# jimouris/draft-mouris-cfrg-mastic

Measured on AMD Instinct MI355X. Metric: VIDPF report x prefix evals/sec at 1/2/4/8 GPUs; % of int-VALU peak, higher is better.
Workload: dtype u32

## Files before the change

draft-mouris-cfrg-mastic_amd/csrc/kernels.hpp:

```cpp
#pragma once
#include "aes.hpp"
#include "flp.hpp"
#include "keccak.hpp"

enum PfxId {
    PFX_EXT = 0,
    PFX_CONV,
    PFX_NODE,
    PFX_ONEHOT,
    PFX_PAYLOAD,
    PFX_EVAL,
    PFX_QUERY,
    PFX_PROOF_SHARE,
    PFX_JR_PART,
    PFX_JR_SEED,
    PFX_JR,
    PFX_PROVE_RAND,
    PFX_TREE,
    PFX_COUNT
};

struct PrefixState {
    KState st;
    int f;
// ... 461 lines not shown
    uint32_t* cache_out;
    int cache_stride;
    uint32_t* wp_buf;
    int recompute_wp;
    int in_stride;
    int fuse_proofs;
    int cur_path_bytes;
    const uint32_t* cur_child_path;
    uint32_t* cur_onehot;
    int pv_level;
    int pv_nodes;
    int pv_npw;
    int pv_path_bytes;
    const uint32_t* pv_child_path;
    uint32_t* pv_onehot;
    int oh_gstride;
    int bin_rstride;
    int pay_gstride;
    const PrefixState* np;
    int np_f;
    int aes_waves;
    int par_waves;
    int proof_prio;
    int aes_prio;
    int dbg_skip;
};

template <class F>
MH_D void parent_payload(const AesPerm& TL, const RkLds& rkc, const uint32_t cv[4], uint32_t t, const uint32_t* cw,
                         int S, int r, int e_lo, int e_hi, uint32_t* out, int row0, int force_slow_blk,
// ... 143 lines not shown
        if (a.proof_prio == 1) __builtin_amdgcn_s_setprio(1);
        if (a.proof_prio == 2) __builtin_amdgcn_s_setprio(2);
        const int nbeg = (blockIdx.y * (EVAL_WAVES - aes_waves) + (wave - aes_waves)) * a.pv_npw;
        const int nend = min(nbeg + a.pv_npw, a.pv_nodes);
        const int pl_ = a.pv_level;
        uint32_t* ohg = a.pv_onehot + (size_t)blockIdx.x * a.oh_gstride;
        const uint32_t lt = (uint32_t)lane * 4u;
        uint32_t pcw[8];
        if constexpr (!WIDE) {
#pragma unroll
            for (int j = 0; j < 8; j++) pcw[j] = pld(pl.cw_proof + ((size_t)pl_ * 8 + j) * S, lb);
        }
        for (int node = nbeg; node < nend; node++) {
            uint32_t sd[4];
#pragma unroll
            for (int i = 0; i < 4; i++) sd[i] = pld(a.cs_in + ((size_t)node * 5 + i) * S_in, lb);
            if constexpr (WIDE) {
                uint32_t w8[8];
                node_proof_one<true>(a.np, a.np_f, p.bits, pl_, a.pv_path_bytes, sd, a.pv_child_path + node * 8, 0u, pcw,
                                     [&](int j, uint32_t w) { w8[j] = w; });
                const uint32_t t = pld(a.cs_in + ((size_t)node * 5 + 4) * S_in, lb);
#pragma unroll
                for (int j = 0; j < 8; j++) pcw[j] = pld(pl.cw_proof + ((size_t)pl_ * 8 + j) * S, lb);
#pragma unroll
                for (int j = 0; j < 8; j++)
                    pst(ohg + ((size_t)node * 8 + j) * a.bin_rstride, lt, w8[j] ^ (t ? pcw[j] : 0u));
            } else {
                const uint32_t t = pld(a.cs_in + ((size_t)node * 5 + 4) * S_in, lb);
                node_proof_one<FC>(a.np, a.np_f, p.bits, pl_, a.pv_path_bytes, sd, a.pv_child_path + node * 8, t, pcw,
                                   [&](int j, uint32_t w) { pst(ohg + ((size_t)node * 8 + j) * a.bin_rstride, lt, w); });
            }
        }
        if (a.proof_prio) __builtin_amdgcn_s_setprio(0);
    }
    const int wp0 = blockIdx.y * a.par_waves * a.ppw;
    const int wp1 = min(wp0 + a.par_waves * a.ppw, SPLIT ? a.n_parents * a.split : a.n_parents);
    const int pn_beg = 2 * wp0, pn_end = 2 * wp1;
    const bool fuse_ovl = FC && a.fuse_proofs == 1;
    auto parent_marked = [&](int q) -> bool {
        const uint32_t w = __hip_atomic_load(parent_done + (q >> 5), __ATOMIC_ACQUIRE, __HIP_MEMORY_SCOPE_WORKGROUP);
        return (__builtin_amdgcn_readfirstlane(w) >> (q & 31)) & 1u;
    };
    auto claim_node = [&]() -> int {
// ... 828 lines not shown
```

draft-mouris-cfrg-mastic_amd/csrc/mastic_hip.hip:

```cpp
#include "mastic_hip.h"

#include <dlfcn.h>
#include <rccl/rccl.h>

#include <algorithm>
#include <atomic>
#include <chrono>
#include <condition_variable>
#include <cstdarg>
#include <cstdio>
#include <cstring>
#include <map>
#include <memory>
#include <mutex>
#include <string>
#include <system_error>
#include <thread>
#include <type_traits>
#include <vector>

#include "comm_agree.hpp"
#include "host_tree.hpp"
#include "kernels.hpp"
#include "shard.hpp"
// ... 158 lines not shown
    int aes_prio = 0;
    int dbg_skip = 0;
    int stride_pad = 64;
    size_t work_arena = (size_t)48 << 30;
    size_t work_arena_fc = (size_t)128 << 30;
    bool binder_tiled = true;
    int absorb_threads = 256;
    int absorb_prio = 3;
    int absorb_dbg = 0;
    int force_slow_blk = -1;
    int fail_allocs = 0;
    int sponge_delay_us = 0;
    int wall_khz = 100000;
    bool timing_nowait = false;
    bool serial_sponges = false;
    bool inject_alloc_failure() {
        if (fail_allocs <= 0) return false;
        fail_allocs--;
        return true;
    }
    bool idle() {
        return hipStreamSynchronize(stream) == hipSuccess && hipStreamSynchronize(stream2) == hipSuccess &&
               hipStreamSynchronize(stream3) == hipSuccess && hipStreamSynchronize(stream4) == hipSuccess;
    }
    int split_sponges = -1;
    bool fuse_last_miss = false;
    bool fuse_last_miss_fc = true;
    bool hit_absorb_main = true;
    bool fc_all = false;
    bool small_split = true;
// ... 430 lines not shown
    const int epb = p.field == 64 ? 2 : 1;
    const int nblk = (p.value_len + epb - 1) / epb;
    const double proofs = 2.0 + (has_prev ? 2.0 * np_prev / std::max(1, np_last) : 0.0);
    const double K = 1585.0 * proofs, A = (4.0 + 2.0 * nblk) * 532.0;
    return std::max(1, std::min(12, (int)std::lround(EVAL_WAVES * K / (K + A))));
}

static int hit_proof_waves(const McParams& p, const mastic_ctx* c) {
    if (c->hit_proof_waves > 0) return c->hit_proof_waves;
    const int epb = p.field == 64 ? 2 : 1;
    const int nblk = (p.value_len + epb - 1) / epb;
    const double K = 3170.0, A = (4.0 + 3.0 * nblk) * 532.0;
    return std::max(1, std::min(12, (int)std::lround(EVAL_WAVES * K / (K + A))));
}

template <class F>
static int run_chunk(mastic_ctx* c, mastic_reports* rep, const Tree* t, const WorkLayout& wl, int agg_id,
                     size_t base, int n, int stride, size_t& evi, LevelCache* lc, bool hit, const uint32_t* cin,
                     uint32_t* cout, uint32_t* W, hipStream_t ss, hipStream_t tail, size_t sev0) {
    const McParams& p = c->p;
    Planes pl = make_planes(W, wl, n, stride);
    Result& R = c->res[agg_id];
    const bool direct = lc && base == 0 && (size_t)n == rep->n && lc->S == (size_t)stride;
    if (direct) {
        pl.sp_onehot = lc->sp.as<uint32_t>();
        pl.sp_payload = lc->sp.as<uint32_t>() + (size_t)50 * lc->S;
        pl.rootsum = lc->rootsum.as<uint32_t>();
    }
    if (hit)
        HIPCHK(c, hipMemsetAsync(pl.status, 0, (size_t)stride * 4, c->stream));
// ... 55 lines not shown
    HIPCHK(c, hipGetLastError());

    const int groups = (n + 63) / 64;
    const int wlw = p.value_len * p.w32;
    int f_oh = c->pfx_f[PFX_ONEHOT], f_pl = c->pfx_f[PFX_PAYLOAD];
    auto plane = [&](size_t off) { return W + off * (size_t)stride; };
    size_t sev = sev0;
    std::vector<hipEvent_t> abs_done(t->L + 1);
    const int oh_gstride = c->binder_tiled ? t->max_level_nodes * 8 * 64 : 64;
    const int pay_gstride = c->binder_tiled ? t->max_parents * wlw * 64 : 64;
    const int bin_rstride = c->binder_tiled ? 64 : stride;
    auto oh_buf = [&](int lv) -> uint32_t* { return plane(wl.onehot[lv % NSLOT]); };
    auto pay_buf = [&](int lv) -> uint32_t* { return plane(wl.payload[lv % NSLOT]); };
    auto oh_gs = [&](int) -> int { return oh_gstride; };
    auto pay_gs = [&](int) -> int { return pay_gstride; };
    const bool pair = c->absorb_mode == 2 || (c->absorb_mode == 0 && (size_t)n < c->absorb_single_min);
    const bool wide = pair && c->eval_wide;
    auto launch_sponges = [&](int lv, int which0, int nwh, hipEvent_t ready, hipEvent_t e4, hipEvent_t e5,
                              hipStream_t as, hipEvent_t* done) -> int {
        AbsorbArgs ab;
        ab.which0 = which0;
        ab.seg[0] = oh_buf(lv);
        ab.gstride[0] = oh_gs(lv);
        ab.nbytes[0] = 2 * t->n_parents[lv] * 32;
        ab.f[0] = f_oh;
        ab.seg[1] = pay_buf(lv);
        ab.gstride[1] = pay_gs(lv);
        ab.rstride = bin_rstride;
        ab.nbytes[1] = lv > 0 ? t->n_parents[lv] * wlw * 4 : 0;
        ab.f[1] = f_pl;
        ab.prio = c->absorb_prio;
        ab.dbg = c->absorb_dbg;
        if (as != c->stream) HIPCHK(c, hipStreamWaitEvent(as, ready, 0));
        if (e4) HIPCHK(c, hipEventRecord(e4, as));
        if (c->dbg_skip & 4) {
        } else if (pair)
            hipLaunchKernelGGL(k_absorb_pair,
                               dim3((groups * 64 * 2 + c->absorb_threads - 1) / c->absorb_threads, (unsigned)nwh),
                               dim3(c->absorb_threads), c->absorb_lds, as, pl, ab);
        else
            hipLaunchKernelGGL(k_absorb, dim3((groups * 64 + 255) / 256, (unsigned)nwh), dim3(256), c->absorb_lds, as,
                               pl, ab);
        if (e5) HIPCHK(c, hipEventRecord(e5, as));
        HIPCHK(c, hipGetLastError());
// ... 23 lines not shown
    if (hit && !direct) {
        if (from_cache(pl.sp_onehot, lc->sp.as<uint32_t>(), 50)) return -1;
        if (from_cache(pl.sp_payload, lc->sp.as<uint32_t>() + (size_t)50 * lc->S, 50)) return -1;
        if (from_cache(pl.rootsum, lc->rootsum.as<uint32_t>(), (size_t)wlw)) return -1;
    }
    if (hit) {
        for (int lv = 0; lv < t->L; lv++) {
            f_oh = (f_oh + 2 * t->n_parents[lv] * 32) % KECCAK_RATE;
            f_pl = (f_pl + (lv > 0 ? t->n_parents[lv] * wlw * 4 : 0)) % KECCAK_RATE;
        }
    }
    const bool fuse_last = hit ? c->fuse_proofs >= 1
                               : ((lc && (c->fuse_proofs == 2 || (c->fuse_proofs >= 1 && c->fuse_last_miss_fc))) ||
                                  (c->fuse_last_miss && c->fuse_proofs >= 1));
    const hipStream_t last_as = (hit && tail == c->stream && c->hit_absorb_main) ? c->stream : ss;
    for (int l = hit ? t->L : 0; l <= t->L; l++) {
        const int np_ = t->n_parents[l];
        if (!hit && l >= NSLOT) {
            HIPCHK(c, hipStreamWaitEvent(c->stream, abs_done[l - NSLOT], 0));
            if (split && pl_done[l - NSLOT]) HIPCHK(c, hipStreamWaitEvent(c->stream, pl_done[l - NSLOT], 0));
        }
        AesArgs a;
        a.level = l;
        a.agg_id = agg_id;
        a.n_parents = np_;
        const int par_waves = c->par_waves > 0 ? c->par_waves : EVAL_WAVES - c->proof_waves;
        a.split = 1;
        a.split_blocks = 0;
        {
            const int epb = p.field == 64 ? 2 : 1;
// ... 31 lines not shown
        if (fuse && a.fuse_proofs == 1)
            a.aes_waves = EVAL_WAVES - (hit ? hit_proof_waves(p, c) : miss_proof_waves(p, c, t->n_parents[l - 1 < 0 ? 0 : l - 1],
                                                                                      np_, l > 0));
        a.par_waves = par_waves;
        a.proof_prio = c->proof_prio;
        a.aes_prio = c->aes_prio;
        a.dbg_skip = c->dbg_skip;
        const int gy = (n_items + a.par_waves * a.ppw - 1) / (a.par_waves * a.ppw);
        a.pv_level = l - 1;
        a.pv_nodes = (l > 0 && !hit) ? 2 * t->n_parents[l - 1] : 0;
        const int pw = EVAL_WAVES - a.aes_waves;
        a.pv_npw = (a.pv_nodes + gy * pw - 1) / (gy * pw);
        a.pv_path_bytes = (l + 7) / 8;
        a.pv_child_path = l > 0 ? t->d_path + t->off[l - 1] * 8 : nullptr;
        a.pv_onehot = l > 0 ? oh_buf(l - 1) : nullptr;
        a.oh_gstride = l > 0 ? oh_gs(l - 1) : oh_gstride;
        a.pay_gstride = pay_gs(l);
        a.bin_rstride = bin_rstride;
        a.np = (const PrefixState*)c->pfx.p + PFX_NODE;
        a.np_f = c->pfx_f[PFX_NODE];
        dim3 grid(groups, gy);
        hipEvent_t e0 = get_event(c, evi++), e1 = get_event(c, evi++);
        hipEvent_t e2 = get_event(c, evi++), e3 = get_event(c, evi++);
        hipEvent_t e4 = get_event(c, evi++), e5 = get_event(c, evi++);
        HIPCHK(c, hipEventRecord(e0, c->stream));
        if ((lc && (hit || l == t->L || c->fc_all)) || fuse)
            hipLaunchKernelGGL((k_eval_aes<F, true, true>), grid, dim3(64 * EVAL_WAVES), EVAL_LDS_BYTES, c->stream,
                               p, pl, a);
        else if (wide && a.split > 1 && l == 0)
            hipLaunchKernelGGL((k_eval_aes_wide<F, true, true>), grid, dim3(64 * EVAL_WAVES), EVAL_LDS_BYTES,
                               c->stream, p, pl, a);
        else if (wide && a.split > 1)
            hipLaunchKernelGGL((k_eval_aes_wide<F, false, true>), grid, dim3(64 * EVAL_WAVES), EVAL_LDS_BYTES,
                               c->stream, p, pl, a);
        else if (wide && (l == 0 || l == t->L))
            hipLaunchKernelGGL((k_eval_aes_wide<F, true>), grid, dim3(64 * EVAL_WAVES), EVAL_LDS_BYTES, c->stream,
                               p, pl, a);
        else if (wide)
            hipLaunchKernelGGL((k_eval_aes_wide<F, false>), grid, dim3(64 * EVAL_WAVES), EVAL_LDS_BYTES, c->stream,
                               p, pl, a);
        else if (a.split > 1 && l == 0)
            hipLaunchKernelGGL((k_eval_aes<F, true, false, true>), grid, dim3(64 * EVAL_WAVES), EVAL_LDS_BYTES,
                               c->stream, p, pl, a);
        else if (a.split > 1)
            hipLaunchKernelGGL((k_eval_aes<F, false, false, true>), grid, dim3(64 * EVAL_WAVES), EVAL_LDS_BYTES,
                               c->stream, p, pl, a);
        else if (l == 0 || l == t->L)
            hipLaunchKernelGGL((k_eval_aes<F, true, false>), grid, dim3(64 * EVAL_WAVES), EVAL_LDS_BYTES, c->stream,
                               p, pl, a);
        else
            hipLaunchKernelGGL((k_eval_aes<F, false, false>), grid, dim3(64 * EVAL_WAVES), EVAL_LDS_BYTES, c->stream,
                               p, pl, a);
        HIPCHK(c, hipEventRecord(e1, c->stream));
        HIPCHK(c, hipGetLastError());
        HIPCHK(c, hipEventRecord(e2, c->stream));
        HIPCHK(c, hipEventRecord(e3, c->stream));
        hipEvent_t aes_done = get_sync_event(c, sev++);
        HIPCHK(c, hipEventRecord(aes_done, c->stream));
        if (split && l > 0) {
            if (launch_sponges(l, 1, 1, aes_done, e4, e5, c->stream3, &pl_done[l])) return -1;
            if (launch_sponges(l - 1, 0, 1, aes_done, nullptr, nullptr, ss, &abs_done[l - 1])) return -1;
        } else if (l > 0 && !hit) {
            if (launch_absorb(l - 1, aes_done, e4, e5, ss)) return -1;
        } else {
            if (c->sponge_delay_us > 0) {
                const unsigned long long ticks =
                    (unsigned long long)c->sponge_delay_us * (unsigned long long)c->wall_khz / 1000;
                c->sponge_delay_us = 0;
                hipLaunchKernelGGL(k_spin, dim3(1), dim3(64), 0, ss, ticks);
                HIPCHK(c, hipGetLastError());
            }
            HIPCHK(c, hipEventRecord(e4, ss));
            HIPCHK(c, hipEventRecord(e5, ss));
        }
    }
    if (fuse_last) {
        const int l = t->L;
        hipEvent_t e0 = get_event(c, evi++), e1 = get_event(c, evi++);
        hipEvent_t e2 = get_event(c, evi++), e3 = get_event(c, evi++);
        hipEvent_t e4 = get_event(c, evi++), e5 = get_event(c, evi++);
        HIPCHK(c, hipEventRecord(e0, c->stream));
        HIPCHK(c, hipEventRecord(e1, c->stream));
        HIPCHK(c, hipEventRecord(e2, c->stream));
        HIPCHK(c, hipEventRecord(e3, c->stream));
        hipEvent_t np_done = get_sync_event(c, sev++);
        HIPCHK(c, hipEventRecord(np_done, c->stream));
        if (split ? launch_sponges(l, 0, 1, np_done, e4, e5, last_as, &abs_done[l])
                  : launch_absorb(l, np_done, e4, e5, last_as))
            return -1;
    } else {
        const int l = t->L;
        const int nn = 2 * t->n_parents[l];
        ProofArgs pa;
        pa.level = l;
        pa.n_nodes = nn;
        pa.npw = choose_ppw(nn, groups);
        pa.path_bytes = (l + 1 + 7) / 8;
        pa.child_path = t->d_path + t->off[l] * 8;
        pa.cs = plane(wl.cs[l & 1]);
        pa.onehot = oh_buf(l);
        pa.oh_gstride = oh_gs(l);
        pa.bin_rstride = bin_rstride;
        pa.np = (const PrefixState*)c->pfx.p + PFX_NODE;
        pa.f = c->pfx_f[PFX_NODE];
        hipEvent_t e0 = get_event(c, evi++), e1 = get_event(c, evi++);
        hipEvent_t e2 = get_event(c, evi++), e3 = get_event(c, evi++);
        hipEvent_t e4 = get_event(c, evi++), e5 = get_event(c, evi++);
        HIPCHK(c, hipEventRecord(e0, c->stream));
        HIPCHK(c, hipEventRecord(e1, c->stream));
        HIPCHK(c, hipEventRecord(e2, c->stream));
        hipLaunchKernelGGL(k_node_proof, dim3(groups, (nn + 4 * pa.npw - 1) / (4 * pa.npw)), dim3(256), 0,
                           c->stream, p, pl, pa);
        HIPCHK(c, hipEventRecord(e3, c->stream));
        HIPCHK(c, hipGetLastError());
        hipEvent_t np_done = get_sync_event(c, sev++);
        HIPCHK(c, hipEventRecord(np_done, c->stream));
        if (split ? launch_sponges(l, 0, 1, np_done, e4, e5, last_as, &abs_done[l])
                  : launch_absorb(l, np_done, e4, e5, last_as))
            return -1;
    }
    hipEvent_t flp_done = nullptr;
    if (t->weight_check) {
        hipEvent_t lv_done = get_sync_event(c, sev++);
        HIPCHK(c, hipEventRecord(lv_done, c->stream));
        HIPCHK(c, hipStreamWaitEvent(c->stream4, lv_done, 0));
        FlpArgs fl{agg_id, t->L};
        hipLaunchKernelGGL(k_flp_rand<F>, dim3((stride + 255) / 256), dim3(256), 0, c->stream4, p, pl, fl, pfx);
        hipLaunchKernelGGL(k_flp_query<F>, dim3((stride + 255) / 256), dim3(256), 0, c->stream4, p, pl,
                           flp_consts<F>(p));
        HIPCHK(c, hipGetLastError());
        flp_done = get_sync_event(c, sev++);
        HIPCHK(c, hipEventRecord(flp_done, c->stream4));
    }
    if (tail != last_as) HIPCHK(c, hipStreamWaitEvent(tail, abs_done[t->L], 0));
    if (split && pl_done[t->L]) HIPCHK(c, hipStreamWaitEvent(tail, pl_done[t->L], 0));
    FinalArgs fa{agg_id, f_oh, f_pl};
    hipLaunchKernelGGL(k_finalize<F>, dim3((stride + 255) / 256), dim3(256), 0, tail, p, pl, fa, pfx);
    HIPCHK(c, hipGetLastError());
    if (flp_done) HIPCHK(c, hipStreamWaitEvent(tail, flp_done, 0));
    if (lc && !direct) {
        if (!hit && to_cache(lc->rootsum.as<uint32_t>(), pl.rootsum, (size_t)wlw)) return -1;
        if (to_cache(lc->sp.as<uint32_t>(), pl.sp_onehot, 50)) return -1;
        if (to_cache(lc->sp.as<uint32_t>() + (size_t)50 * lc->S, pl.sp_payload, 50)) return -1;
    }
    int rc = 0;
    rc |= copy_planes(c, R.eval_proof, R.stride, base, pl.eval_proof, stride, n, 8, tail);
    rc |= copy_planes(c, R.status, R.stride, base, (const uint32_t*)pl.status, stride, n, 1, tail);
    if (t->weight_check) {
        rc |= copy_planes(c, R.verifier, R.stride, base, pl.verifier, stride, n, (size_t)p.verifier_len * p.w32,
                          tail);
// ... 153 lines not shown
            if (c->graveyard.empty() || !c->idle())
                return fail(c, MASTIC_ENOMEM, "out of device memory (work %zu bytes)", want);
            c->bury();
            if (!c->work.ensure(arena) && !c->work.ensure(want))
                return fail(c, MASTIC_ENOMEM, "out of device memory (work %zu bytes)", want);
        }
        chunk = std::min<size_t>(round_up(n, 64), (c->work.bytes / per_report - pad) / 64 * 64);
    }
    if (c->budget) chunk = std::min(chunk, std::max<size_t>(by_budget, 64));
    const bool capped = c->chunk_max > 0 && round_up(c->chunk_max, 64) < chunk;
    if (capped) chunk = round_up(c->chunk_max, 64);
    const size_t half_cap = c->work.bytes / 2 / per_report;
    const bool pipe = c->chunk_pipeline && n > chunk && chunk >= 128 && half_cap >= pad + 64;
    if (pipe) chunk = std::min(capped ? chunk : chunk / 2, half_cap - pad) / 64 * 64;
    const size_t half = c->work.bytes / 2 / 4 / 64 * 64;
    const size_t nsev = 3 * (size_t)t->L + 12;
    size_t evi = 0;
    hipEvent_t t0 = get_event(c, evi++), t1 = get_event(c, evi++);
    HIPCHK(c, hipEventRecord(t0, c->stream));
    hipEvent_t half_free[2] = {get_sync_event(c, 2 * nsev), get_sync_event(c, 2 * nsev + 1)};
    size_t k = 0;
    for (size_t b = 0; b < n; b += chunk, k++) {
        const int nn = (int)std::min(chunk, n - b);
        const int stride = (int)(round_up(nn, 64) + pad);
        const int h = pipe ? (int)(k & 1) : 0;
        if (pipe && k >= 2) HIPCHK(c, hipStreamWaitEvent(c->stream, half_free[h], 0));
        uint32_t* W = c->work.as<uint32_t>() + h * half;
        hipStream_t ss = (pipe && h) ? c->stream3 : c->stream2;
        hipStream_t tail = pipe ? ss : c->stream;
        rc = p.field == 64
                 ? run_chunk<F64>(c, rep, t, wl, agg_id, b, nn, stride, evi, lc, hit, cin, cout, W, ss, tail,
// ... 1079 lines not shown
        if (spl) c->split_sponges = spl[0] == '1' ? 1 : 0;
        const char* flm = getenv("MASTIC_FUSE_LAST_MISS");
        if (flm) c->fuse_last_miss = flm[0] == '1';
        const char* flf = getenv("MASTIC_FUSE_LAST_MISS_FC");
        if (flf) c->fuse_last_miss_fc = flf[0] != '0';
        const char* ham = getenv("MASTIC_HIT_ABSORB_MAIN");
        if (ham) c->hit_absorb_main = ham[0] != '0';
        const char* ssp = getenv("MASTIC_SMALL_SPLIT");
        if (ssp) c->small_split = ssp[0] != '0';
        const char* evw = getenv("MASTIC_EVAL_WIDE");
        if (evw) c->eval_wide = evw[0] != '0';
        const char* tnw = getenv("MASTIC_DBG_TIMING_NOWAIT");
        if (tnw) c->timing_nowait = tnw[0] == '1';
        const char* ssr = getenv("MASTIC_SERIAL_SPONGES");
        if (ssr) c->serial_sponges = ssr[0] == '1';
    }
#endif
    if (hipFuncSetAttribute((const void*)k_eval_aes<F64, false, false>, hipFuncAttributeMaxDynamicSharedMemorySize,
                            EVAL_LDS_BYTES) != hipSuccess ||
        hipFuncSetAttribute((const void*)k_eval_aes<F128, false, false>, hipFuncAttributeMaxDynamicSharedMemorySize,
                            EVAL_LDS_BYTES) != hipSuccess ||
        hipFuncSetAttribute((const void*)k_eval_aes<F64, true, false>, hipFuncAttributeMaxDynamicSharedMemorySize,
                            EVAL_LDS_BYTES) != hipSuccess ||
        hipFuncSetAttribute((const void*)k_eval_aes<F128, true, false>, hipFuncAttributeMaxDynamicSharedMemorySize,
                            EVAL_LDS_BYTES) != hipSuccess ||
        hipFuncSetAttribute((const void*)k_eval_aes<F64, true, true>, hipFuncAttributeMaxDynamicSharedMemorySize,
                            EVAL_LDS_BYTES) != hipSuccess ||
        hipFuncSetAttribute((const void*)k_eval_aes<F128, true, true>, hipFuncAttributeMaxDynamicSharedMemorySize,
                            EVAL_LDS_BYTES) != hipSuccess ||
        hipFuncSetAttribute((const void*)k_eval_aes<F64, true, false, true>,
// ... 80 lines not shown
extern "C" int mastic_set_test_hooks(mastic_ctx* c, int force_slow_blk, int fail_allocs) {
    if (!c) return MASTIC_EINVAL;
    const int pending = c->fail_allocs;
    c->force_slow_blk = force_slow_blk < 0 ? -1 : force_slow_blk;
    c->fail_allocs = std::max(0, fail_allocs);
    return pending;
}

extern "C" int mastic_set_serial_sponges(mastic_ctx* c, int on) {
    if (!c) return MASTIC_EINVAL;
    const int prev = c->serial_sponges ? 1 : 0;
    if (on >= 0) c->serial_sponges = on != 0;
    return prev;
}

extern "C" int mastic_set_test_sponge_delay(mastic_ctx* c, int delay_us) {
    if (!c || delay_us < 0 || delay_us > 10000000) return MASTIC_EINVAL;
    c->sponge_delay_us = delay_us;
    return 0;
}

extern "C" int mastic_abi_version(void) { return MASTIC_ABI_VERSION; }

extern "C" int mastic_set_memory_budget(mastic_ctx* c, uint64_t bytes) {
    if (!c) return MASTIC_EINVAL;
    c->budget = bytes;
    return 0;
}

extern "C" int mastic_get_sizes(const mastic_ctx* c, mastic_sizes* s) {
// ... 21 lines not shown
```

draft-mouris-cfrg-mastic_amd/mastic_amd/_lib.py:

```python
import ctypes
import os
import subprocess
import threading

PKG_DIR = os.path.dirname(os.path.abspath(__file__))
PKG_ROOT = os.path.dirname(PKG_DIR)
REPO_ROOT = os.path.dirname(PKG_ROOT)
CSRC = os.path.join(PKG_ROOT, "csrc")
INCLUDE = os.path.join(REPO_ROOT, "include")
LIB_PATH = os.path.join(PKG_DIR, "libmastic_hip.so")
LOAD_PATH = LIB_PATH
ABI_VERSION = 6

MASTIC_OK = 0
ERRORS = {-22: "EINVAL", -12: "ENOMEM", -19: "ENODEV", -5: "EHIP", -110: "ETIMEDOUT"}

EXPORTS = [
    "mastic_ctx_create", "mastic_ctx_destroy", "mastic_last_error", "mastic_get_sizes",
    "mastic_set_memory_budget", "mastic_reports_create", "mastic_reports_destroy",
    "mastic_reports_count", "mastic_reports_upload", "mastic_reports_download",
    "mastic_reports_shard", "mastic_prep_init", "mastic_prep_result", "mastic_aggregate",
    "mastic_synchronize", "mastic_prep_init_batch", "mastic_decide_batch",
    "mastic_shard_batch", "mastic_last_timing", "mastic_tree_stats", "mastic_fold_shares",
    "mastic_work_bytes", "mastic_last_timing3", "mastic_proof_tree", "mastic_set_frontier_cache",
    "mastic_reports_view", "mastic_decide_results",
    "mastic_aggregate_device_on_stream", "mastic_abi_version", "mastic_set_test_hooks",
    "mastic_set_test_sponge_delay", "mastic_set_serial_sponges",
    "mastic_comm_unique_id", "mastic_comm_init", "mastic_comm_init_timeout", "mastic_comm_info",
    "mastic_comm_destroy",
    "mastic_allgather_fold", "mastic_aggregate_merged", "mastic_merge_host",
]
COMM_ID_BYTES = 128
ROCM_PATH = "/opt/rocm"


class MasticParams(ctypes.Structure):
    _fields_ = [
        ("circuit", ctypes.c_uint32),
        ("bits", ctypes.c_uint32),
        ("length", ctypes.c_uint32),
        ("sum_vec_bits", ctypes.c_uint32),
        ("max_measurement", ctypes.c_uint64),
# ... 87 lines not shown
                                                 ctypes.POINTER(ctypes.c_double)]),
                    "mastic_fold_shares": (i32, [P, P, sz, sz, P, P]),
                    "mastic_comm_unique_id": (i32, [P]),
                    "mastic_comm_init": (i32, [P, i32, i32, P]),
                    "mastic_comm_init_timeout": (i32, [P, i32, i32, P, i32]),
                    "mastic_comm_info": (i32, [P, ctypes.POINTER(ctypes.c_int), ctypes.POINTER(ctypes.c_int)]),
                    "mastic_comm_destroy": (i32, [P]),
                    "mastic_allgather_fold": (i32, [P, P, sz, sz, P, P]),
                    "mastic_aggregate_merged": (i32, [P, ctypes.c_uint32, P, sz, P]),
                    "mastic_merge_host": (i32, [P, P, sz, sz, P]),
                    "mastic_aggregate_device_on_stream": (i32, [P, i32, P, P, P]),
                    "mastic_abi_version": (i32, []),
                    "mastic_set_test_hooks": (i32, [P, i32, i32]),
                    "mastic_set_test_sponge_delay": (i32, [P, i32]),
                    "mastic_set_serial_sponges": (i32, [P, i32]),
                    "mastic_reports_view": (i32, [P, sz, sz, ctypes.POINTER(P)]),
                    "mastic_decide_results": (i32, [P, u8p, sz, P, P]),
                    "mastic_last_timing3": (i32, [P] + [ctypes.POINTER(ctypes.c_double), ctypes.POINTER(ctypes.c_int)] * 3
                                            + [ctypes.POINTER(ctypes.c_double)]),
                    "mastic_work_bytes": (i32, [P, u8p, sz, ctypes.POINTER(ctypes.c_uint64)]),
                    "mastic_proof_tree": (i32, [P, ctypes.c_int, u8p, sz, P, sz]),
                    "mastic_set_frontier_cache": (i32, [P, ctypes.c_int, ctypes.POINTER(ctypes.c_int)]),
                    "mastic_tree_stats": (i32, [P, u8p, sz, ctypes.POINTER(ctypes.c_uint64),
                                                ctypes.POINTER(ctypes.c_uint64), ctypes.POINTER(ctypes.c_uint64)]),
                }
                for name, (res, args) in sig.items():
                    fn = getattr(l, name)
                    fn.restype = res
                    fn.argtypes = args
                if l.mastic_abi_version() != ABI_VERSION:
# ... 19 lines not shown
```

draft-mouris-cfrg-mastic_amd/mastic_amd/vdaf.py:

```python
import ctypes
import itertools

import numpy as np

from . import _lib
from .field import Field64, Field128

PROOF_SIZE = 32
CIRCUIT_IDS = {"Count": 1, "Sum": 2, "SumVec": 3, "Histogram": 4, "MultihotCountVec": 5}


def _check(ctx_ptr, rc):
    if rc != 0:
        msg = _lib.lib().mastic_last_error(ctx_ptr) if ctx_ptr else b""
        text = (msg or b"").decode(errors="replace") or "mastic error"
        if rc == -22:
            raise ValueError(text)
        raise _lib.MasticError(rc, text)


def _pack_path(path) -> bytes:
    return np.packbits(np.fromiter(path, dtype=bool, count=len(path))).tobytes()


# ... 303 lines not shown
    def set_test_hooks(self, force_slow_blk: int = -1, fail_allocs: int = 0):
        rc = _lib.lib().mastic_set_test_hooks(self._ctx, int(force_slow_blk), int(fail_allocs))
        if rc < 0:
            _check(self._ctx, rc)
        return rc

    def set_test_sponge_delay(self, delay_us: int):
        _check(self._ctx, _lib.lib().mastic_set_test_sponge_delay(self._ctx, int(delay_us)))

    def set_serial_sponges(self, on=None) -> bool:
        rc = _lib.lib().mastic_set_serial_sponges(self._ctx, -1 if on is None else int(bool(on)))
        if rc < 0:
            _check(self._ctx, rc)
        return bool(rc)

    def set_frontier_cache(self, on: bool):
        _check(self._ctx, _lib.lib().mastic_set_frontier_cache(self._ctx, 1 if on else 0, None))

    def last_prep_was_cached(self) -> bool:
        v = ctypes.c_int()
        _check(self._ctx, _lib.lib().mastic_set_frontier_cache(self._ctx, -1, ctypes.byref(v)))
        return bool(v.value)

    def proof_tree(self, agg_id: int, ctx: bytes, n: int):
        from .proof_agg import level_sizes
        sizes = level_sizes(n)
        out = np.empty(32 * max(1, sum(sizes)), np.uint8)
        _check(self._ctx, _lib.lib().mastic_proof_tree(self._ctx, agg_id, ctx, len(ctx), _lib.buf(out), sum(sizes)))
        raw = out.tobytes()
        levels, off = [], 0
# ... 293 lines not shown
```

include/mastic_hip.h:

```cpp
#ifndef MASTIC_HIP_H
#define MASTIC_HIP_H

#include <stddef.h>
#include <stdint.h>

#ifdef __cplusplus
extern "C" {
#endif

#define MASTIC_ABI_VERSION 6

#define MASTIC_OK 0
#define MASTIC_EINVAL (-22)
#define MASTIC_ENOMEM (-12)
#define MASTIC_ENODEV (-19)
#define MASTIC_EHIP (-5)
#define MASTIC_ETIMEDOUT (-110)

#define MASTIC_COUNT 1
#define MASTIC_SUM 2
#define MASTIC_SUMVEC 3
#define MASTIC_HISTOGRAM 4
#define MASTIC_MULTIHOT 5

typedef struct mastic_params {
// ... 61 lines not shown
int mastic_comm_init(mastic_ctx* ctx, int nranks, int rank, const uint8_t id[MASTIC_COMM_ID_BYTES]);
int mastic_comm_init_timeout(mastic_ctx* ctx, int nranks, int rank, const uint8_t id[MASTIC_COMM_ID_BYTES],
                             int timeout_ms);
int mastic_comm_info(const mastic_ctx* ctx, int* nranks, int* rank);
int mastic_comm_destroy(mastic_ctx* ctx);
int mastic_allgather_fold(mastic_ctx* ctx, const void* dev_local, size_t n_local, size_t n_elems, void* dev_out,
                          void* caller_stream);
int mastic_merge_host(mastic_ctx* ctx, const uint8_t* host_local, size_t n_local, size_t n_elems, uint8_t* host_out);
#define MASTIC_MERGE_ZEROS 4u
int mastic_aggregate_merged(mastic_ctx* ctx, uint32_t agg_mask, const uint8_t* valid, size_t n_elems,
                            uint8_t* agg_out);
int mastic_proof_tree(mastic_ctx* ctx, int agg_id, const uint8_t* app_ctx, size_t ctx_len, uint8_t* nodes_out,
                      size_t n_nodes);
int mastic_set_frontier_cache(mastic_ctx* ctx, int on, int* last_hit);
int mastic_set_serial_sponges(mastic_ctx* ctx, int on);
int mastic_synchronize(mastic_ctx* ctx);
int mastic_abi_version(void);
int mastic_set_test_hooks(mastic_ctx* ctx, int force_slow_blk, int fail_allocs);
int mastic_set_test_sponge_delay(mastic_ctx* ctx, int delay_us);

int mastic_prep_init_batch(mastic_ctx* ctx, const uint8_t* verify_key, size_t verify_key_len,
                           const uint8_t* app_ctx, size_t ctx_len, int agg_id, const uint8_t* enc_agg_param, size_t agg_param_len, size_t n,
                           const uint8_t* nonces, const uint8_t* public_shares, const uint8_t* input_shares,
                           uint8_t* prep_shares_out, uint8_t* jr_seeds_out, uint8_t* out_shares_out,
                           int32_t* status_out);

#define MASTIC_DECIDE_VIDPF_FAIL 0
#define MASTIC_DECIDE_OK 1
#define MASTIC_DECIDE_FLP_FAIL 2
int mastic_decide_batch(mastic_ctx* ctx, const uint8_t* app_ctx, size_t ctx_len, const uint8_t* enc_agg_param,
// ... 20 lines not shown
```

integration/poc/mastic_hip.py:

```python
import ctypes

ABI_VERSION = 6
_EINVAL = -22
PROOF_SIZE = 32
DECIDE_VIDPF_FAIL, DECIDE_OK, DECIDE_FLP_FAIL = 0, 1, 2


class MasticParams(ctypes.Structure):
    _fields_ = [("circuit", ctypes.c_uint32), ("bits", ctypes.c_uint32), ("length", ctypes.c_uint32),
                ("sum_vec_bits", ctypes.c_uint32), ("max_measurement", ctypes.c_uint64),
                ("chunk_length", ctypes.c_uint32), ("device", ctypes.c_int32)]


class MasticSizes(ctypes.Structure):
    _fields_ = [(name, ctypes.c_uint32) for name in (
        "field_bytes", "value_len", "meas_len", "output_len", "proof_len", "verifier_len",
        "joint_rand_len", "query_rand_len", "prove_rand_len", "rand_size", "public_share_size")] + [
        ("input_share_size", ctypes.c_uint32 * 2),
        ("prep_share_size", ctypes.c_uint32 * 2),
        ("algorithm_id", ctypes.c_uint32),
    ]


def load(path="libmastic_hip.so"):
# ... 139 lines not shown
```

Before: 140.9 million.

## Segment last tree level to overlap eval, node proofs and sponge absorbs

Splits the last VIDPF level into several geometrically balanced parent segments, launched as separate eval kernels. Each segment's kernel computes the node proofs of the previous segment and launches partial one-hot and payload sponge absorbs on side streams, so hashing overlaps with the remaining AES work instead of waiting for the whole level. The payload absorb of the second-to-last level is also started earlier. The cost is more kernel launches, events and partial sponge passes, plus the risk of underfilling the GPU on small segments, which an auto-selection heuristic tries to avoid.

Result: faster. 142.7 million, median of 6 (+1.3%).

```diff
diff --git a/draft-mouris-cfrg-mastic_amd/csrc/kernels.hpp b/draft-mouris-cfrg-mastic_amd/csrc/kernels.hpp
--- a/draft-mouris-cfrg-mastic_amd/csrc/kernels.hpp
+++ b/draft-mouris-cfrg-mastic_amd/csrc/kernels.hpp
@@ -499,6 +499,7 @@
     int pv_path_bytes;
     const uint32_t* pv_child_path;
     uint32_t* pv_onehot;
+    const uint32_t* pv_cs;
     int oh_gstride;
     int bin_rstride;
     int pay_gstride;
@@ -672,19 +673,19 @@
         for (int node = nbeg; node < nend; node++) {
             uint32_t sd[4];
 #pragma unroll
-            for (int i = 0; i < 4; i++) sd[i] = pld(a.cs_in + ((size_t)node * 5 + i) * S_in, lb);
+            for (int i = 0; i < 4; i++) sd[i] = pld(a.pv_cs + ((size_t)node * 5 + i) * S, lb);
             if constexpr (WIDE) {
                 uint32_t w8[8];
                 node_proof_one<true>(a.np, a.np_f, p.bits, pl_, a.pv_path_bytes, sd, a.pv_child_path + node * 8, 0u, pcw,
                                      [&](int j, uint32_t w) { w8[j] = w; });
-                const uint32_t t = pld(a.cs_in + ((size_t)node * 5 + 4) * S_in, lb);
+                const uint32_t t = pld(a.pv_cs + ((size_t)node * 5 + 4) * S, lb);
 #pragma unroll
                 for (int j = 0; j < 8; j++) pcw[j] = pld(pl.cw_proof + ((size_t)pl_ * 8 + j) * S, lb);
 #pragma unroll
                 for (int j = 0; j < 8; j++)
                     pst(ohg + ((size_t)node * 8 + j) * a.bin_rstride, lt, w8[j] ^ (t ? pcw[j] : 0u));
             } else {
-                const uint32_t t = pld(a.cs_in + ((size_t)node * 5 + 4) * S_in, lb);
+                const uint32_t t = pld(a.pv_cs + ((size_t)node * 5 + 4) * S, lb);
                 node_proof_one<FC>(a.np, a.np_f, p.bits, pl_, a.pv_path_bytes, sd, a.pv_child_path + node * 8, t, pcw,
                                    [&](int j, uint32_t w) { pst(ohg + ((size_t)node * 8 + j) * a.bin_rstride, lt, w); });
             }
diff --git a/draft-mouris-cfrg-mastic_amd/csrc/mastic_hip.hip b/draft-mouris-cfrg-mastic_amd/csrc/mastic_hip.hip
--- a/draft-mouris-cfrg-mastic_amd/csrc/mastic_hip.hip
+++ b/draft-mouris-cfrg-mastic_amd/csrc/mastic_hip.hip
@@ -196,6 +196,9 @@
     int wall_khz = 100000;
     bool timing_nowait = false;
     bool serial_sponges = false;
+    int last_level_segments = 0;
+    bool seg_early_payload = true;
+    bool seg_balance = true;
     bool inject_alloc_failure() {
         if (fail_allocs <= 0) return false;
         fail_allocs--;
@@ -656,6 +659,53 @@
     return std::max(1, std::min(12, (int)std::lround(EVAL_WAVES * K / (K + A))));
 }
 
+static std::vector<int> segment_ranges(const mastic_ctx* c, const Tree* t, int k) {
+    const int npl = t->n_parents[t->L];
+    std::vector<int> beg(k + 1, 0);
+    beg[k] = npl;
+    if (k <= 1) return beg;
+    const double prev = (double)t->n_parents[t->L - 1];
+    std::vector<double> sz(k, (double)npl / k);
+    if (c->seg_balance) {
+        double lo = 0.0, hi = 1.0 + (double)npl / prev;
+        for (int it = 0; it < 60; it++) {
+            const double y = 0.5 * (lo + hi);
+            double sum = 0.0, last = prev;
+            for (int q = 0; q < k; q++) {
+                sz[q] = last * y;
+                last = sz[q];
+                sum += sz[q];
+            }
+            (sum < npl ? lo : hi) = y;
+        }
+    }
+    double acc = 0.0;
+    for (int q = 1; q < k; q++) {
+        acc += sz[q - 1];
+        beg[q] = std::max(beg[q - 1] + 1, std::min((int)std::lround(acc), npl - (k - q)));
+    }
+    return beg;
+}
+
+static constexpr int LAST_LEVEL_SEGMENTS_AUTO = 4;
+static int last_level_segments(const mastic_ctx* c, const Tree* t, int groups, int par_waves) {
+    const int np = t->n_parents[t->L];
+    if (c->last_level_segments >= 1) return std::max(1, std::min(c->last_level_segments, np));
+    int k = std::min(LAST_LEVEL_SEGMENTS_AUTO, np);
+    for (; k > 1; k /= 2) {
+        const std::vector<int> beg = segment_ranges(c, t, k);
+        bool fills = true;
+        for (int q = 0; q < k && fills; q++) {
+            const int cnt = beg[q + 1] - beg[q];
+            const int ppw = choose_eval_ppw(cnt, groups, par_waves, c->n_cus);
+            const long long gy = (cnt + (long long)par_waves * ppw - 1) / ((long long)par_waves * ppw);
+            fills = groups * gy >= 2LL * c->n_cus;
+        }
+        if (fills) break;
+    }
+    return std::max(1, k);
+}
+
 template <class F>
 static int run_chunk(mastic_ctx* c, mastic_reports* rep, const Tree* t, const WorkLayout& wl, int agg_id,
                      size_t base, int n, int stride, size_t& evi, LevelCache* lc, bool hit, const uint32_t* cin,
@@ -741,20 +791,26 @@
     auto pay_buf = [&](int lv) -> uint32_t* { return plane(wl.payload[lv % NSLOT]); };
     auto oh_gs = [&](int) -> int { return oh_gstride; };
     auto pay_gs = [&](int) -> int { return pay_gstride; };
+    struct Piece {
+        int node0, nodes;
+        int parent0, parents;
+    };
     const bool pair = c->absorb_mode == 2 || (c->absorb_mode == 0 && (size_t)n < c->absorb_single_min);
     const bool wide = pair && c->eval_wide;
     auto launch_sponges = [&](int lv, int which0, int nwh, hipEvent_t ready, hipEvent_t e4, hipEvent_t e5,
-                              hipStream_t as, hipEvent_t* done) -> int {
+                              hipStream_t as, hipEvent_t* done, const Piece* piece = nullptr) -> int {
+        const Piece whole{0, 2 * t->n_parents[lv], 0, t->n_parents[lv]};
+        const Piece& pc = piece ? *piece : whole;
         AbsorbArgs ab;
         ab.which0 = which0;
-        ab.seg[0] = oh_buf(lv);
+        ab.seg[0] = oh_buf(lv) + (size_t)pc.node0 * 8 * bin_rstride;
         ab.gstride[0] = oh_gs(lv);
-        ab.nbytes[0] = 2 * t->n_parents[lv] * 32;
+        ab.nbytes[0] = pc.nodes * 32;
         ab.f[0] = f_oh;
-        ab.seg[1] = pay_buf(lv);
+        ab.seg[1] = pay_buf(lv) + (size_t)pc.parent0 * wlw * bin_rstride;
         ab.gstride[1] = pay_gs(lv);
         ab.rstride = bin_rstride;
-        ab.nbytes[1] = lv > 0 ? t->n_parents[lv] * wlw * 4 : 0;
+        ab.nbytes[1] = lv > 0 ? pc.parents * wlw * 4 : 0;
         ab.f[1] = f_pl;
         ab.prio = c->absorb_prio;
         ab.dbg = c->absorb_dbg;
@@ -808,6 +864,49 @@
                                : ((lc && (c->fuse_proofs == 2 || (c->fuse_proofs >= 1 && c->fuse_last_miss_fc))) ||
                                   (c->fuse_last_miss && c->fuse_proofs >= 1));
     const hipStream_t last_as = (hit && tail == c->stream && c->hit_absorb_main) ? c->stream : ss;
+    const int L_ = t->L;
+    int nseg = 1;
+    if (!lc && !hit && tail == c->stream && ss == c->stream2 && pair && !fuse_last) {
+        const int par_waves = c->par_waves > 0 ? c->par_waves : EVAL_WAVES - c->proof_waves;
+        nseg = last_level_segments(c, t, groups, par_waves);
+    }
+    const bool seg_early = nseg > 1 && c->seg_early_payload && !split && L_ >= 2;
+    const std::vector<int> seg_beg = segment_ranges(c, t, nseg);
+    auto piece_marks = [&](hipStream_t as, hipEvent_t* e4, hipEvent_t* e5) -> int {
+        for (int i = 0; i < 4; i++) HIPCHK(c, hipEventRecord(get_event(c, evi++), as));
+        *e4 = get_event(c, evi++);
+        *e5 = get_event(c, evi++);
+        return 0;
+    };
+    auto launch_level = [&](const AesArgs& a, dim3 grid, int l, bool fuse) {
+        if ((lc && (hit || l == t->L || c->fc_all)) || fuse)
+            hipLaunchKernelGGL((k_eval_aes<F, true, true>), grid, dim3(64 * EVAL_WAVES), EVAL_LDS_BYTES, c->stream,
+                               p, pl, a);
+        else if (wide && a.split > 1 && l == 0)
+            hipLaunchKernelGGL((k_eval_aes_wide<F, true, true>), grid, dim3(64 * EVAL_WAVES), EVAL_LDS_BYTES,
+                               c->stream, p, pl, a);
+        else if (wide && a.split > 1)
+            hipLaunchKernelGGL((k_eval_aes_wide<F, false, true>), grid, dim3(64 * EVAL_WAVES), EVAL_LDS_BYTES,
+                               c->stream, p, pl, a);
+        else if (wide && (l == 0 || l == t->L))
+            hipLaunchKernelGGL((k_eval_aes_wide<F, true>), grid, dim3(64 * EVAL_WAVES), EVAL_LDS_BYTES, c->stream,
+                               p, pl, a);
+        else if (wide)
+            hipLaunchKernelGGL((k_eval_aes_wide<F, false>), grid, dim3(64 * EVAL_WAVES), EVAL_LDS_BYTES, c->stream,
+                               p, pl, a);
+        else if (a.split > 1 && l == 0)
+            hipLaunchKernelGGL((k_eval_aes<F, true, false, true>), grid, dim3(64 * EVAL_WAVES), EVAL_LDS_BYTES,
+                               c->stream, p, pl, a);
+        else if (a.split > 1)
+            hipLaunchKernelGGL((k_eval_aes<F, false, false, true>), grid, dim3(64 * EVAL_WAVES), EVAL_LDS_BYTES,
+                               c->stream, p, pl, a);
+        else if (l == 0 || l == t->L)
+            hipLaunchKernelGGL((k_eval_aes<F, true, false>), grid, dim3(64 * EVAL_WAVES), EVAL_LDS_BYTES, c->stream,
+                               p, pl, a);
+        else
+            hipLaunchKernelGGL((k_eval_aes<F, false, false>), grid, dim3(64 * EVAL_WAVES), EVAL_LDS_BYTES, c->stream,
+                               p, pl, a);
+    };
     for (int l = hit ? t->L : 0; l <= t->L; l++) {
         const int np_ = t->n_parents[l];
         if (!hit && l >= NSLOT) {
@@ -869,43 +968,70 @@
         a.pv_path_bytes = (l + 7) / 8;
         a.pv_child_path = l > 0 ? t->d_path + t->off[l - 1] * 8 : nullptr;
         a.pv_onehot = l > 0 ? oh_buf(l - 1) : nullptr;
+        a.pv_cs = a.cs_in;
         a.oh_gstride = l > 0 ? oh_gs(l - 1) : oh_gstride;
         a.pay_gstride = pay_gs(l);
         a.bin_rstride = bin_rstride;
         a.np = (const PrefixState*)c->pfx.p + PFX_NODE;
         a.np_f = c->pfx_f[PFX_NODE];
+        if (nseg > 1 && l == L_) {
+            for (int q = 0; q < nseg; q++) {
+                const int p0 = seg_beg[q], cnt = seg_beg[q + 1] - p0;
+                AesArgs b = a;
+                b.n_parents = cnt;
+                b.ppw = choose_eval_ppw(cnt, groups, par_waves, c->n_cus);
+                b.parent_node = a.parent_node + p0;
+                b.child_exp = a.child_exp + 2 * (size_t)p0;
+                b.child_pfx = a.child_pfx + 2 * (size_t)p0;
+                b.cur_child_path = a.cur_child_path + 2 * (size_t)p0 * 8;
+                b.cs_out = a.cs_out + 2 * (size_t)p0 * 5 * stride;
+                b.fr_w_in = a.fr_w_in + (size_t)p0 * wlw * stride;
+                b.payload = a.payload + (size_t)p0 * wlw * bin_rstride;
+                if (q > 0) {
+                    const size_t n0 = 2 * (size_t)seg_beg[q - 1];
+                    b.pv_level = l;
+                    b.pv_nodes = 2 * (p0 - seg_beg[q - 1]);
+                    b.pv_path_bytes = (l + 1 + 7) / 8;
+                    b.pv_child_path = t->d_path + (t->off[l] + n0) * 8;
+                    b.pv_onehot = oh_buf(l) + n0 * 8 * bin_rstride;
+                    b.pv_cs = a.cs_out + n0 * 5 * stride;
+                    b.oh_gstride = oh_gs(l);
+                }
+                const int gyq = (cnt + b.par_waves * b.ppw - 1) / (b.par_waves * b.ppw);
+                b.pv_npw = (b.pv_nodes + gyq * pw - 1) / (gyq * pw);
+                hipEvent_t e0 = get_event(c, evi++), e1 = get_event(c, evi++);
+                hipEvent_t e2 = get_event(c, evi++), e3 = get_event(c, evi++);
+                hipEvent_t e4 = get_event(c, evi++), e5 = get_event(c, evi++);
+                HIPCHK(c, hipEventRecord(e0, c->stream));
+                launch_level(b, dim3(groups, gyq), l, false);
+                HIPCHK(c, hipEventRecord(e1, c->stream));
+                HIPCHK(c, hipGetLastError());
+                HIPCHK(c, hipEventRecord(e2, c->stream));
+                HIPCHK(c, hipEventRecord(e3, c->stream));
+                hipEvent_t aes_done = get_sync_event(c, sev++);
+                HIPCHK(c, hipEventRecord(aes_done, c->stream));
+                if (q > 0) {
+                    const Piece pc{2 * seg_beg[q - 1], 2 * (p0 - seg_beg[q - 1]), 0, 0};
+                    if (launch_sponges(l, 0, 1, aes_done, e4, e5, ss, &abs_done[l], &pc)) return -1;
+                } else if (split || seg_early) {
+                    if (launch_sponges(l - 1, 0, 1, aes_done, e4, e5, ss, &abs_done[l - 1])) return -1;
+                } else {
+                    if (launch_absorb(l - 1, aes_done, e4, e5, ss)) return -1;
+                    HIPCHK(c, hipStreamWaitEvent(c->stream3, abs_done[l - 1], 0));
+                }
+                hipEvent_t p4, p5;
+                if (piece_marks(c->stream3, &p4, &p5)) return -1;
+                const Piece pp{0, 0, p0, cnt};
+                if (launch_sponges(l, 1, 1, aes_done, p4, p5, c->stream3, &pl_done[l], &pp)) return -1;
+            }
+            continue;
+        }
         dim3 grid(groups, gy);
         hipEvent_t e0 = get_event(c, evi++), e1 = get_event(c, evi++);
         hipEvent_t e2 = get_event(c, evi++), e3 = get_event(c, evi++);
         hipEvent_t e4 = get_event(c, evi++), e5 = get_event(c, evi++);
         HIPCHK(c, hipEventRecord(e0, c->stream));
-        if ((lc && (hit || l == t->L || c->fc_all)) || fuse)
-            hipLaunchKernelGGL((k_eval_aes<F, true, true>), grid, dim3(64 * EVAL_WAVES), EVAL_LDS_BYTES, c->stream,
-                               p, pl, a);
-        else if (wide && a.split > 1 && l == 0)
-            hipLaunchKernelGGL((k_eval_aes_wide<F, true, true>), grid, dim3(64 * EVAL_WAVES), EVAL_LDS_BYTES,
-                               c->stream, p, pl, a);
-        else if (wide && a.split > 1)
-            hipLaunchKernelGGL((k_eval_aes_wide<F, false, true>), grid, dim3(64 * EVAL_WAVES), EVAL_LDS_BYTES,
-                               c->stream, p, pl, a);
-        else if (wide && (l == 0 || l == t->L))
-            hipLaunchKernelGGL((k_eval_aes_wide<F, true>), grid, dim3(64 * EVAL_WAVES), EVAL_LDS_BYTES, c->stream,
-                               p, pl, a);
-        else if (wide)
-            hipLaunchKernelGGL((k_eval_aes_wide<F, false>), grid, dim3(64 * EVAL_WAVES), EVAL_LDS_BYTES, c->stream,
-                               p, pl, a);
-        else if (a.split > 1 && l == 0)
-            hipLaunchKernelGGL((k_eval_aes<F, true, false, true>), grid, dim3(64 * EVAL_WAVES), EVAL_LDS_BYTES,
-                               c->stream, p, pl, a);
-        else if (a.split > 1)
-            hipLaunchKernelGGL((k_eval_aes<F, false, false, true>), grid, dim3(64 * EVAL_WAVES), EVAL_LDS_BYTES,
-                               c->stream, p, pl, a);
-        else if (l == 0 || l == t->L)
-            hipLaunchKernelGGL((k_eval_aes<F, true, false>), grid, dim3(64 * EVAL_WAVES), EVAL_LDS_BYTES, c->stream,
-                               p, pl, a);
-        else
-            hipLaunchKernelGGL((k_eval_aes<F, false, false>), grid, dim3(64 * EVAL_WAVES), EVAL_LDS_BYTES, c->stream,
-                               p, pl, a);
+        launch_level(a, grid, l, fuse);
         HIPCHK(c, hipEventRecord(e1, c->stream));
         HIPCHK(c, hipGetLastError());
         HIPCHK(c, hipEventRecord(e2, c->stream));
@@ -917,6 +1043,12 @@
             if (launch_sponges(l - 1, 0, 1, aes_done, nullptr, nullptr, ss, &abs_done[l - 1])) return -1;
         } else if (l > 0 && !hit) {
             if (launch_absorb(l - 1, aes_done, e4, e5, ss)) return -1;
+            if (seg_early && l == L_ - 1) {
+                hipEvent_t p4, p5;
+                HIPCHK(c, hipStreamWaitEvent(c->stream3, abs_done[l - 1], 0));
+                if (piece_marks(c->stream3, &p4, &p5)) return -1;
+                if (launch_sponges(l, 1, 1, aes_done, p4, p5, c->stream3, &pl_done[l])) return -1;
+            }
         } else {
             if (c->sponge_delay_us > 0) {
                 const unsigned long long ticks =
@@ -945,15 +1077,16 @@
             return -1;
     } else {
         const int l = t->L;
-        const int nn = 2 * t->n_parents[l];
+        const int n0 = 2 * seg_beg[nseg - 1];
+        const int nn = 2 * t->n_parents[l] - n0;
         ProofArgs pa;
         pa.level = l;
         pa.n_nodes = nn;
         pa.npw = choose_ppw(nn, groups);
         pa.path_bytes = (l + 1 + 7) / 8;
-        pa.child_path = t->d_path + t->off[l] * 8;
-        pa.cs = plane(wl.cs[l & 1]);
-        pa.onehot = oh_buf(l);
+        pa.child_path = t->d_path + (t->off[l] + (size_t)n0) * 8;
+        pa.cs = plane(wl.cs[l & 1]) + (size_t)n0 * 5 * stride;
+        pa.onehot = oh_buf(l) + (size_t)n0 * 8 * bin_rstride;
         pa.oh_gstride = oh_gs(l);
         pa.bin_rstride = bin_rstride;
         pa.np = (const PrefixState*)c->pfx.p + PFX_NODE;
@@ -970,8 +1103,10 @@
         HIPCHK(c, hipGetLastError());
         hipEvent_t np_done = get_sync_event(c, sev++);
         HIPCHK(c, hipEventRecord(np_done, c->stream));
-        if (split ? launch_sponges(l, 0, 1, np_done, e4, e5, last_as, &abs_done[l])
-                  : launch_absorb(l, np_done, e4, e5, last_as))
+        const Piece pc{n0, nn, 0, 0};
+        if (nseg > 1 ? launch_sponges(l, 0, 1, np_done, e4, e5, last_as, &abs_done[l], &pc)
+            : split  ? launch_sponges(l, 0, 1, np_done, e4, e5, last_as, &abs_done[l])
+                     : launch_absorb(l, np_done, e4, e5, last_as))
             return -1;
     }
     hipEvent_t flp_done = nullptr;
@@ -988,7 +1123,7 @@
         HIPCHK(c, hipEventRecord(flp_done, c->stream4));
     }
     if (tail != last_as) HIPCHK(c, hipStreamWaitEvent(tail, abs_done[t->L], 0));
-    if (split && pl_done[t->L]) HIPCHK(c, hipStreamWaitEvent(tail, pl_done[t->L], 0));
+    if (pl_done[t->L]) HIPCHK(c, hipStreamWaitEvent(tail, pl_done[t->L], 0));
     FinalArgs fa{agg_id, f_oh, f_pl};
     hipLaunchKernelGGL(k_finalize<F>, dim3((stride + 255) / 256), dim3(256), 0, tail, p, pl, fa, pfx);
     HIPCHK(c, hipGetLastError());
@@ -1172,7 +1307,8 @@
     const bool pipe = c->chunk_pipeline && n > chunk && chunk >= 128 && half_cap >= pad + 64;
     if (pipe) chunk = std::min(capped ? chunk : chunk / 2, half_cap - pad) / 64 * 64;
     const size_t half = c->work.bytes / 2 / 4 / 64 * 64;
-    const size_t nsev = 3 * (size_t)t->L + 12;
+    const size_t nsev = 3 * (size_t)t->L + 12 +
+                        3 * (size_t)std::min(std::max(c->last_level_segments, LAST_LEVEL_SEGMENTS_AUTO), t->n_parents[t->L]);
     size_t evi = 0;
     hipEvent_t t0 = get_event(c, evi++), t1 = get_event(c, evi++);
     HIPCHK(c, hipEventRecord(t0, c->stream));
@@ -2282,6 +2418,12 @@
         if (tnw) c->timing_nowait = tnw[0] == '1';
         const char* ssr = getenv("MASTIC_SERIAL_SPONGES");
         if (ssr) c->serial_sponges = ssr[0] == '1';
+        const char* lls = getenv("MASTIC_LAST_LEVEL_SEGMENTS");
+        if (lls) c->last_level_segments = std::max(0, atoi(lls));
+        const char* sge = getenv("MASTIC_SEG_EARLY");
+        if (sge) c->seg_early_payload = sge[0] != '0';
+        const char* sgb = getenv("MASTIC_SEG_BALANCE");
+        if (sgb) c->seg_balance = sgb[0] != '0';
     }
 #endif
     if (hipFuncSetAttribute((const void*)k_eval_aes<F64, false, false>, hipFuncAttributeMaxDynamicSharedMemorySize,
@@ -2392,6 +2534,13 @@
     return prev;
 }
 
+extern "C" int mastic_set_last_level_segments(mastic_ctx* c, int k) {
+    if (!c || k < 0) return MASTIC_EINVAL;
+    const int prev = c->last_level_segments;
+    c->last_level_segments = k;
+    return prev;
+}
+
 extern "C" int mastic_set_test_sponge_delay(mastic_ctx* c, int delay_us) {
     if (!c || delay_us < 0 || delay_us > 10000000) return MASTIC_EINVAL;
     c->sponge_delay_us = delay_us;
diff --git a/draft-mouris-cfrg-mastic_amd/mastic_amd/_lib.py b/draft-mouris-cfrg-mastic_amd/mastic_amd/_lib.py
--- a/draft-mouris-cfrg-mastic_amd/mastic_amd/_lib.py
+++ b/draft-mouris-cfrg-mastic_amd/mastic_amd/_lib.py
@@ -10,7 +10,7 @@
 INCLUDE = os.path.join(REPO_ROOT, "include")
 LIB_PATH = os.path.join(PKG_DIR, "libmastic_hip.so")
 LOAD_PATH = LIB_PATH
-ABI_VERSION = 6
+ABI_VERSION = 7
 
 MASTIC_OK = 0
 ERRORS = {-22: "EINVAL", -12: "ENOMEM", -19: "ENODEV", -5: "EHIP", -110: "ETIMEDOUT"}
@@ -25,7 +25,7 @@
     "mastic_work_bytes", "mastic_last_timing3", "mastic_proof_tree", "mastic_set_frontier_cache",
     "mastic_reports_view", "mastic_decide_results",
     "mastic_aggregate_device_on_stream", "mastic_abi_version", "mastic_set_test_hooks",
-    "mastic_set_test_sponge_delay", "mastic_set_serial_sponges",
+    "mastic_set_test_sponge_delay", "mastic_set_serial_sponges", "mastic_set_last_level_segments",
     "mastic_comm_unique_id", "mastic_comm_init", "mastic_comm_init_timeout", "mastic_comm_info",
     "mastic_comm_destroy",
     "mastic_allgather_fold", "mastic_aggregate_merged", "mastic_merge_host",
@@ -143,6 +143,7 @@
                     "mastic_set_test_hooks": (i32, [P, i32, i32]),
                     "mastic_set_test_sponge_delay": (i32, [P, i32]),
                     "mastic_set_serial_sponges": (i32, [P, i32]),
+                    "mastic_set_last_level_segments": (i32, [P, i32]),
                     "mastic_reports_view": (i32, [P, sz, sz, ctypes.POINTER(P)]),
                     "mastic_decide_results": (i32, [P, u8p, sz, P, P]),
                     "mastic_last_timing3": (i32, [P] + [ctypes.POINTER(ctypes.c_double), ctypes.POINTER(ctypes.c_int)] * 3
diff --git a/draft-mouris-cfrg-mastic_amd/mastic_amd/vdaf.py b/draft-mouris-cfrg-mastic_amd/mastic_amd/vdaf.py
--- a/draft-mouris-cfrg-mastic_amd/mastic_amd/vdaf.py
+++ b/draft-mouris-cfrg-mastic_amd/mastic_amd/vdaf.py
@@ -341,6 +341,12 @@
             _check(self._ctx, rc)
         return bool(rc)
 
+    def set_last_level_segments(self, k: int = 0) -> int:
+        rc = _lib.lib().mastic_set_last_level_segments(self._ctx, int(k))
+        if rc < 0:
+            _check(self._ctx, rc)
+        return rc
+
     def set_frontier_cache(self, on: bool):
         _check(self._ctx, _lib.lib().mastic_set_frontier_cache(self._ctx, 1 if on else 0, None))
 
diff --git a/include/mastic_hip.h b/include/mastic_hip.h
--- a/include/mastic_hip.h
+++ b/include/mastic_hip.h
@@ -8,7 +8,7 @@
 extern "C" {
 #endif
 
-#define MASTIC_ABI_VERSION 6
+#define MASTIC_ABI_VERSION 7
 
 #define MASTIC_OK 0
 #define MASTIC_EINVAL (-22)
@@ -100,6 +100,7 @@
                       size_t n_nodes);
 int mastic_set_frontier_cache(mastic_ctx* ctx, int on, int* last_hit);
 int mastic_set_serial_sponges(mastic_ctx* ctx, int on);
+int mastic_set_last_level_segments(mastic_ctx* ctx, int k);
 int mastic_synchronize(mastic_ctx* ctx);
 int mastic_abi_version(void);
 int mastic_set_test_hooks(mastic_ctx* ctx, int force_slow_blk, int fail_allocs);
diff --git a/integration/poc/mastic_hip.py b/integration/poc/mastic_hip.py
--- a/integration/poc/mastic_hip.py
+++ b/integration/poc/mastic_hip.py
@@ -1,6 +1,6 @@
 import ctypes
 
-ABI_VERSION = 6
+ABI_VERSION = 7
 _EINVAL = -22
 PROOF_SIZE = 32
 DECIDE_VIDPF_FAIL, DECIDE_OK, DECIDE_FLP_FAIL = 0, 1, 2
```
